# myshell-ai/OpenVoice

Hardware: NVIDIA H100
Metric: audio_seconds_per_second (higher is better)
Workload: dtype f32 (3xFP16 split-precision tensor-core convs with fp32 accumulation, fp32 FFMA elsewhere)

## Files before the change

### openvoice_b200/csrc/ovc_lib.cu

```cuda
#include <cuda_runtime.h>

#include <algorithm>
#include <cmath>
#include <cstdarg>
#include <cstdio>
#include <cstdlib>
#include <cstring>
#include <map>
#include <string>
#include <vector>

#include "../../include/ovc.h"
#include "ovc_convpack.h"
#include "ovc_small.cuh"
#include "ovc_tcconv.cuh"
#include "ovc_tts.cuh"
#include "ovc_refenc.cuh"
#include "ovc_resample.cuh"
#include "ovc_splice.h"
#include "ovc_variants.h"

namespace ovc {

static thread_local std::string g_err;
// ... 116 lines not shown

}

using namespace ovc;

struct ovc_ctx {
  ovc_hparams hp{};
  int device = 0;
  int sm_count = 0;
  std::map<std::string, HostTensor> sd;
  bool finalized = false;

  float* d_w = nullptr;
  size_t w_floats = 0;
  std::vector<float> h_w;

  ConvLayer enc_pre, enc_pre16, enc_proj;
  WNLayers enc_wn;
  ConvLayer flow_pre[4], flow_post[4];
  WNLayers flow_wn[4];
  ConvLayer dec_pre, dec_ups[4];
  ConvLayer rb_c1[12][3], rb_c2[12][3];
  TcLayer tc_c1[12][3], tc_c2[12][3], tc_ups[4], tc_pre;
  float* d_tcw = nullptr;
  std::vector<float> h_tcw;
  int precision = 0;
  bool tts_simple = false;
  bool use_graph = true;
  int use_pdl = 2;
  bool use_branches = true;
  int par_frames = 512;
  bool use_pair = true;
  bool use_pair_occ = true;
  bool use_staged_epi = true;
  bool pair_occ2_ok[TCN_N_OCC2] = {};
  cudaStream_t br_stream[2] = {nullptr, nullptr};
  cudaEvent_t br_ev[4] = {nullptr, nullptr, nullptr, nullptr};
  size_t post_w_off = 0;
  size_t cond_w_off = 0, cond_b_off = 0;
  int* d_cond_wrow = nullptr;
  int* d_cond_sel = nullptr;
  int cond_rows_out = 0;
  int cond_off_enc = 0, cond_off_fsrc = 0, cond_off_ftgt = 0, cond_off_dec = 0;
  int cond_off_enc_tc = 0, cond_off_fsrc_tc = 0, cond_off_ftgt_tc = 0;
  int* d_cond_cols[2][3] = {};
  int cond_pf_cols[2][3] = {};
  int cond_pf_off[2][3][4] = {};

  float2* d_tw = nullptr;
  float* d_win = nullptr;

  bool has_refenc = false;
  size_t re_conv_w[6] = {0}, re_conv_b[6] = {0}, re_wih = 0, re_whh = 0, re_bih = 0, re_bhh = 0, re_pw = 0, re_pb = 0,
         re_lng = 0, re_lnb = 0;
  int re_gru_in = 0;
  float* d_re = nullptr;
  size_t re_floats = 0;
  float* d_res = nullptr;
  size_t res_floats = 0;

  std::map<std::pair<int64_t, int64_t>, double*> rs_banks;
  bool rs_smem_opt_in = false;
  std::vector<RsRingPlan> rs_plans;
  RsRingPlan* d_rs_plans = nullptr;
  int rs_ring_tile = 256;
  size_t rs_ring_smem = 0;

// ... 627 lines not shown
  cfg.dynamicSmemBytes = smem;
  cfg.stream = st;
  cudaLaunchAttribute at[1];
  at[0].id = cudaLaunchAttributeProgrammaticStreamSerialization;
  at[0].val.programmaticStreamSerializationAllowed = 1;
  cfg.attrs = at;
  cfg.numAttrs = pdl ? 1 : 0;
  return cudaLaunchKernelEx(&cfg, kernel, std::forward<Args>(args)...);
}

static int launch_tc(Run& r, const TcLayer& T, const float* x, float* y, const float* res, int t_len, int mul, float slope,
                     float scale, int accumulate, int family, const TcExtra& ex = TcExtra()) {
  TcConvArgs a{};
  const int y_ld = ex.y_ld ? ex.y_ld : T.Ntot;
  a.x = x; a.x_bs = (long long)T.Cin * r.P * mul;
  a.w = reinterpret_cast<const uint16_t*>(r.c->d_tcw + T.w_off);
  a.bias = ex.bias ? ex.bias : r.c->d_tcw + T.b_off; a.bias_bs = ex.bias_bs; a.bias_ts = ex.bias_ts;
  a.y = y; a.y_bs = (long long)y_ld * r.P * mul; a.y_ld = y_ld;
  a.r = res;
  a.s = ex.s; a.s_bs = a.y_bs;
  a.epi = ex.epi; a.split = ex.split; a.first = ex.first;
  a.lens = ex.use_lens_frames ? r.lens : r.glens; a.tmax = r.Tmax; a.mul = mul;
  a.lens_x = ex.lens_x; a.has_lens_x = ex.has_lens_x ? 1 : 0;
  a.Cin = T.Cin; a.Ntot = T.Ntot; a.K = T.K; a.DIL = T.DIL;
  a.slope = slope; a.scale = scale; a.accumulate = accumulate;
  a.passes = r.c->precision == 2 ? 1 : 3;
  if (T.TN == 0) return fail(OVC_ERR_INVALID, "conv %d -> %d (k %d, dilation %d) does not fit the tensor-core kernels", T.Cin, T.Ntot, T.K, T.DIL);
  if (!(slope >= 0.f && slope <= 1.f)) return fail(OVC_ERR_INVALID, "leaky_relu slope %g outside [0, 1]", (double)slope);
  TRY(prof_begin(r));
  const TcGrid g = tc_grid(t_len, r.B, T.Ntot, T.TN, r.c->sm_count, ex.grid_div);
  const int n_tt = g.n_tt, total = g.total;
  dim3 pg((unsigned)g.grid_x, g.ncol, 1);
  const bool pdl = r.c->use_pdl == 1 || (r.c->use_pdl == 2 && ex.epi != 0);
  const TcKernel k = tc_conv_kernel(T.TN, r.c->use_staged_epi && tc_stage_pays(T.K, a.passes));
  CK(launch_ex(k.fn, pg, k.threads, k.smem, r.st, pdl, a, n_tt, total));
  CK(cudaGetLastError());
  r.c->launches++;
  const double units = (double)r.B * t_len;
  const int eff_k = family == 2 ? 2 : T.K;
  TRY(prof_end(r, T.TN == 128 ? V_TC128 : T.TN == 64 ? V_TC64 : V_TC32, family == 1 ? 1 : 0, 2.0 * T.Cin * T.Ntot * eff_k * units,
               4.0 * (T.Cin + T.Ntot * (1 + (res ? 1 : 0) + (accumulate ? 1 : 0))) * units, (T.Cin << 16) | (T.K << 8) | T.DIL));
  return OVC_OK;
}

static int launch_pair(Run& r, const TcLayer& T1, const TcLayer& T2, const float* x, float* y, int t_len, int mul, float slope,
                       float scale, int accumulate) {
  TcConvArgs a{};
  const int C = T1.TN;
  a.x = x; a.x_bs = (long long)C * r.P * mul;
  a.w = reinterpret_cast<const uint16_t*>(r.c->d_tcw + T1.w_off);
  a.w2 = reinterpret_cast<const uint16_t*>(r.c->d_tcw + T2.w_off);
  a.bias = r.c->d_tcw + T1.b_off; a.bias2 = r.c->d_tcw + T2.b_off;
  a.y = y; a.y_bs = a.x_bs; a.y_ld = C;
  a.lens = r.glens; a.tmax = r.Tmax; a.mul = mul;
  a.Cin = C; a.Ntot = C; a.K = T1.K; a.DIL = T1.DIL;
  a.slope = slope; a.scale = scale; a.accumulate = accumulate;
  a.passes = r.c->precision == 2 ? 1 : 3;
  TcPairOcc o = r.c->use_pair_occ ? tc_pair_occ(T1, T2) : TcPairOcc();
  for (int i = 0; i < TCN_N_OCC2; ++i)
    if (o.occ == 2 && kTcPairOcc2[i].C == C && kTcPairOcc2[i].o.nabuf == o.nabuf && !r.c->pair_occ2_ok[i]) o = TcPairOcc();
  const TcKernel k = tc_pair_kernel(C, o, r.c->use_staged_epi && tc_stage_pays(T1.K, a.passes));
  if (!k.fn) return fail(OVC_ERR_INVALID, "no conv-pair kernel for C = %d at %d CTA(s) per SM, %d operand buffer(s)", C, o.occ, o.nabuf);
  const TcGrid g = tc_pair_grid(t_len, r.B, T1.K, r.c->sm_count, o.occ);
  const int n_tt = g.n_tt, total = g.total;
  TRY(prof_begin(r));
  dim3 pg((unsigned)g.grid_x, 1, 1);
  CK(launch_ex(k.fn, pg, k.threads, k.smem, r.st, false, a, n_tt, total));
  CK(cudaGetLastError());
  r.c->launches++;
  const double units = (double)r.B * t_len;
  TRY(prof_end(r, C == 128 ? V_TCPAIR128 : C == 64 ? V_TCPAIR64 : V_TCPAIR32, 1, 2.0 * 2.0 * C * C * T1.K * units, 4.0 * C * (2 + (accumulate ? 1 : 0)) * units,
               (C << 16) | (T1.K << 8) | T1.DIL));
  return OVC_OK;
}

static int launch_transpose(Run& r, const float* src, float* dst, int rows, int cols) {
  dim3 grid((cols + 31) / 32, (rows + 31) / 32, r.B);
  TRY(prof_begin(r));
  transpose_kernel<<<grid, 256, 0, r.st>>>(src, dst, rows, cols, (long long)rows * cols);
  CK(cudaGetLastError());
  r.c->launches++;
  TRY(prof_end(r, V_TRANSPOSE, 0, 0.0, 8.0 * rows * cols * r.B));
  return OVC_OK;
}

struct CondRef {
  const float* p; long long bs, ts;
  CondRef at(int col) const { return {p + col, bs, ts}; }
};

static int run_wn(Run& r, const WNLayers& wn, float* x, float* skip, float* acts, const CondRef& cond) {
  const int P = r.P, T = r.Tmax;
  const long long bs = 192LL * P;
  const int n = (int)wn.in.size();
// ... 1253 lines not shown
  if (!dst || dst_rows < 1 || dst_cap < 1)
    return fail(OVC_ERR_INVALID, "ovc_splice: bad destination (rows %lld, cap %lld)", (long long)dst_rows, (long long)dst_cap);
  if (src_rows < 0 || (src_rows > 0 && (!src || src_pitch < 1)))
    return fail(OVC_ERR_INVALID, "ovc_splice: bad source (rows %lld, pitch %lld)", (long long)src_rows, (long long)src_pitch);
  if (flags & ~(OVC_SPLICE_PCM16 | OVC_SPLICE_SRC_WRAP)) return fail(OVC_ERR_INVALID, "ovc_splice: unknown flags %d", flags);
  if (S == 0) return OVC_OK;
  const int gy = S < 65535 ? S : 65535;
  const int gx = std::max(1, std::min(1024, 2048 / gy));
  ovc_sp::splice_kernel<<<dim3(gx, gy), 256, 0, (cudaStream_t)stream>>>(src, src_rows, src_pitch, seg, S, dst, dst_rows,
                                                                         dst_cap, flags);
  CK(cudaGetLastError());
  return OVC_OK;
}

int ovc_set_precision(ovc_ctx* c, int mode) {
  if (!c) return fail(OVC_ERR_INVALID, "null context");
  if (mode < 0 || mode > 2) return fail(OVC_ERR_INVALID, "precision mode must be 0 (fp32 FFMA), 1 (3xFP16 tensor cores) or 2 (single-pass fp16)");
  c->precision = mode;
  return OVC_OK;
}

int ovc_set_option(ovc_ctx* c, int key, int value) {
  if (!c) return fail(OVC_ERR_INVALID, "null context");
  switch (key) {
    case OVC_OPT_TTS_SIMPLE: c->tts_simple = value != 0; return OVC_OK;
    case OVC_OPT_GRAPH: c->use_graph = value != 0; return OVC_OK;
    case OVC_OPT_PDL:
      if (value < 0 || value > 2) return fail(OVC_ERR_INVALID, "pdl must be 0, 1 or 2");
      c->use_pdl = value;
      return OVC_OK;
    case OVC_OPT_BRANCHES: c->use_branches = value != 0; return OVC_OK;
    case OVC_OPT_PAIR: c->use_pair = value != 0; return OVC_OK;
    case OVC_OPT_PAIR_OCC: c->use_pair_occ = value != 0; return OVC_OK;
    case OVC_OPT_STAGED_EPI: c->use_staged_epi = value != 0; return OVC_OK;
    default: return fail(OVC_ERR_INVALID, "unknown option %d", key);
  }
}

int ovc_last_launch_count(const ovc_ctx* c) { return c ? c->launches : 0; }

int ovc_graph_replays(const ovc_ctx* c) { return c ? c->graph_replays : 0; }

int ovc_profile_enable(ovc_ctx* c, int enable) {
  if (!c) return fail(OVC_ERR_INVALID, "null context");
  c->prof = enable != 0;
  c->ev_used = 0;
  c->ev_flops.clear();
  c->ev_bytes.clear();
  c->ev_variant.clear();
  c->ev_family.clear();
  c->ev_tag.clear();
  return OVC_OK;
}

int ovc_profile_read(ovc_ctx* c, double* ms, int64_t* launches, double* flops, double* bytes) {
  if (!c) return fail(OVC_ERR_INVALID, "null context");
  double tms = 0, tf = 0, tb = 0;
  int64_t n = 0;
  for (size_t i = 0; i + 1 < c->ev_used; i += 2) {
    if (!c->ev_family[i / 2]) continue;
    float m = 0;
    CK(cudaEventElapsedTime(&m, c->ev[i], c->ev[i + 1]));
    tms += m;
    tf += c->ev_flops[i / 2];
    tb += c->ev_bytes[i / 2];
    ++n;
  }
// ... 58 lines not shown
```

### openvoice_b200/csrc/ovc_tcconv.cuh

```cuda
#pragma once
#include "ovc_conv.cuh"
#include "ovc_tc.cuh"
#include "ovc_tcpack.h"

namespace ovc {

struct TcConvArgs {
  const float* x; long long x_bs;
  const uint16_t* w;
  const float* bias; long long bias_bs;
  float* y; long long y_bs; int y_ld;
  const float* r;
  float* s; long long s_bs;
  int epi;
  int split; int first;
  const long long* lens; int tmax; int mul;
  const long long* lens_x; int has_lens_x;
  int Cin; int Ntot; int K; int DIL;
  float slope; float scale; int accumulate;
  int passes;
  const uint16_t* w2; const float* bias2;
  long long bias_ts;
};

// ... 66 lines not shown
      for (int g = 0; g < 2; ++g) {
        const float2 oa = make_float2(tanhf(v[4 * g]) * sigmoidf_acc(v[4 * (g + 2)]),
                                      tanhf(v[4 * g + 1]) * sigmoidf_acc(v[4 * (g + 2) + 1]));
        const float2 ob = make_float2(tanhf(v[4 * g + 2]) * sigmoidf_acc(v[4 * (g + 2) + 2]),
                                      tanhf(v[4 * g + 3]) * sigmoidf_acc(v[4 * (g + 2) + 3]));
        if (oka) *reinterpret_cast<float2*>(ypa + 8 * g) = oa;
        if (okb) *reinterpret_cast<float2*>(ypb + 8 * g) = ob;
      }
    } else {
      const int col = n0 + c0;
      const bool to_x = col < a.split;
      const bool add = to_x || !a.first;
      float* dst = (to_x ? yb + col : sb + (col - a.split)) + csub;
#pragma unroll
      for (int g = 0; g < 4; ++g) {
        float2 oa = make_float2(v[4 * g], v[4 * g + 1]), ob = make_float2(v[4 * g + 2], v[4 * g + 3]);
        if (add) {
          const float2 qa = oka ? *reinterpret_cast<const float2*>(dst + (size_t)ta * a.y_ld + 8 * g) : make_float2(0.f, 0.f);
          const float2 qb = okb ? *reinterpret_cast<const float2*>(dst + (size_t)tb * a.y_ld + 8 * g) : make_float2(0.f, 0.f);
          oa = make_float2(qa.x + oa.x, qa.y + oa.y);
          ob = make_float2(qb.x + ob.x, qb.y + ob.y);
        }
        if (oka) *reinterpret_cast<float2*>(dst + (size_t)ta * a.y_ld + 8 * g) = oa;
        if (okb) *reinterpret_cast<float2*>(dst + (size_t)tb * a.y_ld + 8 * g) = ob;
      }
    }
  }
}

template <int TN, class V>
__device__ __forceinline__ void tc_epilogue_v(const TcConvArgs& a, V v_at, int b, int t0, int n0, int lim, int row_a) {
  if (a.bias_ts) tc_epilogue_body<TN, true>(a, v_at, b, t0, n0, lim, row_a);
  else tc_epilogue_body<TN, false>(a, v_at, b, t0, n0, lim, row_a);
}

template <int TN>
__device__ __forceinline__ void tc_epilogue(const TcConvArgs& a, const float (&d)[TN], int b, int t0, int n0, int lim, int row_a) {
  const bool two = a.passes == 3;
  tc_epilogue_v<TN>(a, [&](int j) { return tc_result<TN>(d, two, j); }, b, t0, n0, lim, row_a);
}
__device__ __forceinline__ TcConvArgs tc_pair_epilogue_args(const TcConvArgs& a, int TN) {
  TcConvArgs e = a;
  e.y_ld = TN; e.r = a.x; e.bias = a.bias2; e.bias_bs = 0; e.bias_ts = 0; e.epi = 0;
  return e;
}

template <int TN>
__device__ __forceinline__ void tc_mma_step(float (&d)[TN], uint64_t a_hi, uint64_t a_lo, uint64_t b, bool three, bool first) {
  float (&lo)[TN / 2] = *reinterpret_cast<float(*)[TN / 2]>(&d[TN / 2]);
  float (&hi)[TN / 2] = *reinterpret_cast<float(*)[TN / 2]>(&d[0]);
  tc::Wgmma<TN>::mma(hi, a_hi, b, first ? 0 : 1);
  if (three) {
    tc::Wgmma<TN>::mma(lo, a_hi, b + TN, first ? 0 : 1);
    tc::Wgmma<TN>::mma(lo, a_lo, b, 1);
  }
}

constexpr int TCN_THREADS = 384;
constexpr int TCN_NCT = 96;

template <int TN, bool PAIR, int OCC = 1, int NAB = 2, bool STAGED = false>
struct TcnCfg {
  static_assert(!PAIR || TN == 32 || TN == 64 || TN == 128, "conv pairs: C = 32, 64 or 128");
  static_assert(OCC == 1 || (PAIR && TN <= 64), "two CTAs per SM: C = 32 / 64 pairs");
  static_assert(!STAGED || (TN == 128 && OCC == 1), "staged epilogue: TN = 128, one CTA per SM");
  static constexpr int THREADS = STAGED ? TCN_THREADS + 128 : TCN_THREADS;
  static constexpr int KCH = 32, NKC = KCH / 8;
  static constexpr int ROWS = 194;
  static constexpr int ROWS2 = TCN_ROWS2;
  static constexpr int NABUF = NAB;
  static constexpr int RING = PAIR ? tc_pair_ring(TN, OCC, NAB) : tc_ring_slots(TN, PAIR);
  static constexpr int SLOT_BYTES = 2 * 2 * TN * 16;
  static constexpr int A_BUF_BYTES = 2 * NKC * ROWS * 16;
  static constexpr int A2_BYTES = PAIR ? 2 * (TN / 8) * ROWS2 * 16 : 0;
  static constexpr int STAGE_BYTES = STAGED ? (TN / 2) * 256 * 4 : 0;
  static_assert(!STAGED || !PAIR || STAGE_BYTES <= A2_BYTES, "a pair's staging tile lies in its conv-2 operand");
  static constexpr int SBUF_BYTES = STAGED && !PAIR ? STAGE_BYTES : 0;
  static constexpr size_t SMEM_BYTES = 1024 + NABUF * A_BUF_BYTES + A2_BYTES + RING * SLOT_BYTES + SBUF_BYTES;
  static_assert(!PAIR || SMEM_BYTES == tc_pair_smem(TN, NABUF, RING), "tc_pair_smem");
  static_assert(SMEM_BYTES <= (OCC == 1 ? 232448 : TCN_SMEM_OCC2), "shared memory budget");
  static_assert((2 * NABUF + 2 * RING + 2) * 8 <= 1024, "barrier area");
  static constexpr int PROD_REGS = OCC == 1 && !STAGED ? 56 : 32, MMA_REGS = STAGED ? 184 : OCC == 1 ? 224 : 104;
  static constexpr int STORE_REGS = 112;
  static_assert(128 * PROD_REGS + 256 * MMA_REGS + (STAGED ? 128 * STORE_REGS : 0) <= 65536 / OCC, "register budget");
};

template <int TN, bool PAIR, int OCC = 1, int NAB = 2, bool STAGED = false>
__global__ void __launch_bounds__(TcnCfg<TN, PAIR, OCC, NAB, STAGED>::THREADS, OCC) tcconv_kernel(const TcConvArgs a, int n_tt, int total) {
  using Cfg = TcnCfg<TN, PAIR, OCC, NAB, STAGED>;
  constexpr int ROWS = Cfg::ROWS, ROWS2 = Cfg::ROWS2, NABUF = Cfg::NABUF, RING = Cfg::RING, NKC = Cfg::NKC;
  extern __shared__ __align__(128) unsigned char smem_raw[];
  uint64_t* bars = reinterpret_cast<uint64_t*>(smem_raw);
  uint64_t *a_full = bars, *a_empty = bars + NABUF, *b_full = a_empty + NABUF, *b_empty = b_full + RING;
  uint64_t *s_full = b_empty + RING, *s_empty = s_full + 1;
  unsigned char* abuf = smem_raw + 1024;
  unsigned char* a2buf = abuf + NABUF * Cfg::A_BUF_BYTES;
  unsigned char* bring = a2buf + Cfg::A2_BYTES;
  float* stage = reinterpret_cast<float*>(PAIR ? a2buf : bring + RING * Cfg::SLOT_BYTES);

  const int tid = threadIdx.x, lane = tid & 31;
  const int warp = __shfl_sync(0xffffffffu, tid >> 5, 0);
  const int H1 = (a.K - 1) / 2 * a.DIL;
  const int H2 = PAIR ? (a.K - 1) / 2 : 0;
  const int R = 128 - 2 * H2;
  const int rows8 = (128 + 2 * H1 + 7) & ~7;
  const int nq = a.Cin / Cfg::KCH;
  const int n_slots = (a.Cin / 16) * a.K;
  const int n_w = PAIR ? 2 * n_slots : n_slots;
  const bool resident = n_w <= RING;
  if (H1 > TCN_HMAX || (PAIR && 128 + 2 * H2 > ROWS2)) __trap();
  constexpr uint32_t BYTES = Cfg::SLOT_BYTES;

  if (tid == 0) {
    for (int i = 0; i < NABUF; ++i) { mbar_init(&a_full[i], TCN_NCT); mbar_init(&a_empty[i], 2); }
    for (int i = 0; i < RING; ++i) { mbar_init(&b_full[i], 1); mbar_init(&b_empty[i], 2); }
    if (STAGED) { mbar_init(s_full, 256); mbar_init(s_empty, 128); }
    fence_mbar_init();
  }
  if (PAIR) {
    for (int i = tid; i < Cfg::A2_BYTES / 16; i += Cfg::THREADS) reinterpret_cast<uint4*>(a2buf)[i] = make_uint4(0u, 0u, 0u, 0u);
// ... 15 lines not shown
    tc::regs_dealloc<Cfg::PROD_REGS>();
    if (warp == 0) {
      if (lane == 0) {
        const unsigned char* wt = reinterpret_cast<const unsigned char*>(a.w) + (size_t)blockIdx.y * n_slots * BYTES;
        if (resident) {
          for (int it = 0; it < n_w; ++it) {
            const unsigned char* src = it < n_slots ? wt + (size_t)it * BYTES
                                                    : reinterpret_cast<const unsigned char*>(a.w2) + (size_t)(it - n_slots) * BYTES;
            mbar_expect_tx(&b_full[it], BYTES);
            tma_bulk_g2s(bring + it * BYTES, src, BYTES, &b_full[it]);
          }
          for (int it = 0; it < n_w; ++it) mbar_wait(&b_full[it], 0u);
        } else {
          int slot = 0;
          uint32_t phase = 1;
          TCN_FOR_TILES
            (void)b;
            for (int it = 0; it < n_w; ++it) {
              const unsigned char* src = it < n_slots ? wt + (size_t)it * BYTES
                                                      : reinterpret_cast<const unsigned char*>(a.w2) + (size_t)(it - n_slots) * BYTES;
              mbar_wait(&b_empty[slot], phase);
              mbar_expect_tx(&b_full[slot], BYTES);
              tma_bulk_g2s(bring + slot * BYTES, src, BYTES, &b_full[slot]);
              if (++slot == RING) { slot = 0; phase ^= 1; }
            }
          }
        }
      }
    } else {
      const int pt = tid - 32;
      const int items = rows8 * NKC;
      int buf = 0;
      uint32_t ephase = 1;
      TCN_FOR_TILES
        const float* xb = a.x + (size_t)b * a.x_bs;
        const int r0 = t0 - H2 - H1;
        for (int q = 0; q < nq; ++q) {
          mbar_wait(&a_empty[buf], ephase);
          unsigned char* ah = abuf + buf * Cfg::A_BUF_BYTES;
          unsigned char* al = ah + NKC * ROWS * 16;
          constexpr int PB = 2;
          for (int i0 = pt; i0 < items; i0 += TCN_NCT * PB) {
            float4 v0[PB], v1[PB];
#pragma unroll
            for (int u = 0; u < PB; ++u) {
              const int i = i0 + TCN_NCT * u;
              const int row = i >> 2, kc = i & 3;
              const int t = r0 + row;
              v0[u] = make_float4(0.f, 0.f, 0.f, 0.f);
              v1[u] = v0[u];
              if (i < items && t >= 0 && t < lim_x) {
                const float4* src = reinterpret_cast<const float4*>(xb + (size_t)t * a.Cin + q * Cfg::KCH + kc * 8);
                v0[u] = src[0];
                v1[u] = src[1];
              }
            }
#pragma unroll
            for (int u = 0; u < PB; ++u) {
              const int i = i0 + TCN_NCT * u;
              if (i >= items) break;
              const int row = i >> 2, kc = i & 3;
              uint4 hi, lo;
              tc::split_f16x8(v0[u], v1[u], a.slope, hi, lo);
              *reinterpret_cast<uint4*>(ah + (kc * ROWS + row) * 16) = hi;
              *reinterpret_cast<uint4*>(al + (kc * ROWS + row) * 16) = lo;
            }
          }
          asm volatile("fence.proxy.async.shared::cta;" ::: "memory");
          mbar_arrive(&a_full[buf]);
          if (++buf == NABUF) { buf = 0; ephase ^= 1; }
        }
      }
    }
  } else if (STAGED && warp >= 12) {
    tc::regs_dealloc<Cfg::STORE_REGS>();
    const int st = tid & 127;
    uint32_t phase = 0;
    TCN_FOR_TILES
      if (PAIR) named_bar_arrive(1, 384);
      mbar_wait(s_full, phase);
      phase ^= 1;
#pragma unroll 1
      for (int h = 0; h < 2; ++h) {
        const float* sv = stage + h * 128 + st;
        const auto v_at = [&](int j) { return sv[j * 256]; };
        const int row_a = 64 * h + 16 * (warp & 3) + (lane >> 2);
        if constexpr (PAIR) tc_epilogue_v<TN>(tc_pair_epilogue_args(a, TN), v_at, b, t0, 0, min(lim, t0 + R), row_a);
        else tc_epilogue_v<TN>(a, v_at, b, t0, blockIdx.y * TN, lim, row_a);
      }
      if (!PAIR) mbar_arrive(s_empty);
    }
  } else {
    tc::regs_alloc<Cfg::MMA_REGS>();
    const int wg = (warp >> 2) - 1;
    const bool leader = (tid & 127) == 0;
    const int row_a = 64 * wg + 16 * (warp & 3) + (lane >> 2);
    constexpr uint32_t LBO_A = ROWS * 16, LBO_A2 = ROWS2 * 16, LBO_B = 2 * TN * 16, SBO = 128;
    constexpr uint32_t A_LO16 = (NKC * ROWS * 16) >> 4, A2_LO16 = ((TN / 8) * ROWS2 * 16) >> 4, SLOT16 = BYTES >> 4;
    const uint64_t a_proto = tc::make_desc(0, LBO_A, SBO), b_proto = tc::make_desc(0, LBO_B, SBO);
    const uint64_t b_ring = b_proto + (tc::smem_addr(bring) >> 4);
    const bool three = a.passes == 3;
    float d[TN];
#pragma unroll
    for (int i = 0; i < TN; ++i) d[i] = 0.f;
    const auto stage_tile = [&]() {
#pragma unroll
      for (int j = 0; j < TN / 2; ++j) stage[j * 256 + tid - 128] = tc_result<TN>(d, three, j);
      mbar_arrive(s_full);
    };
    uint32_t sphase = 1;
    (void)sphase;
    if (resident)
      for (int it = 0; it < n_w; ++it) mbar_wait(&b_full[it], 0u);
    int slot = 0, buf = 0;
    uint32_t bphase = 0, aphase = 0;
    TCN_FOR_TILES
      (void)lim_x;
      bool first = true;
      if (resident) slot = 0;
      for (int q = 0; q < nq; ++q) {
        mbar_wait(&a_full[buf], aphase);
// ... 76 lines not shown
              tc_mma_step<TN>(d, a_cur, a_cur + A2_LO16, b_ring + (uint32_t)slot * SLOT16, three, first2);
              tc::wgmma_commit();
              tc::wgmma_wait<1>();
              if (leader && prev >= 0) mbar_arrive(&b_empty[prev]);
              prev = slot;
              if (++slot == RING) { slot = 0; bphase ^= 1; }
            }
            first2 = false;
            a_cur += 1;
          }
        }
        tc::wgmma_commit();
        tc::wgmma_wait<0>();
        tc::fence_regs(d);
        if (leader && prev >= 0) mbar_arrive(&b_empty[prev]);
        if constexpr (STAGED) {
          named_bar_sync(3, 256);
          stage_tile();
        } else {
          tc_epilogue<TN>(tc_pair_epilogue_args(a, TN), d, b, t0, 0, min(lim, t0 + R), row_a);
        }
      }
    }
  }
#undef TCN_FOR_TILES
}

struct TcKernel {
  void (*fn)(TcConvArgs, int, int) = nullptr;
  size_t smem = 0;
  int threads = 0;
};
using TcPairKernel = TcKernel;
template <int TN, bool PAIR, int OCC = 1, int NAB = 2, bool STAGED = false>
inline TcKernel tc_kernel() {
  using Cfg = TcnCfg<TN, PAIR, OCC, NAB, STAGED>;
  return {tcconv_kernel<TN, PAIR, OCC, NAB, STAGED>, Cfg::SMEM_BYTES, Cfg::THREADS};
}
inline bool tc_stage_pays(int K, int passes) { return passes * K >= 15; }
inline TcKernel tc_conv_kernel(int TN, bool staged) {
  if (TN == 128) return staged ? tc_kernel<128, false, 1, 2, true>() : tc_kernel<128, false>();
  if (TN == 64) return tc_kernel<64, false>();
  if (TN == 32) return tc_kernel<32, false>();
  return {};
}
inline TcKernel tc_pair_kernel(int C, TcPairOcc o, bool staged = false) {
  if (o.occ == 1 && o.nabuf == 2) {
    if (C == 128) return staged ? tc_kernel<128, true, 1, 2, true>() : tc_kernel<128, true>();
    if (C == 64) return tc_kernel<64, true>();
    if (C == 32) return tc_kernel<32, true>();
  } else if (o.occ == 2) {
    if (C == 32 && o.nabuf == 2) return tc_kernel<32, true, 2, 2>();
    if (C == 32 && o.nabuf == 1) return tc_kernel<32, true, 2, 1>();
    if (C == 64 && o.nabuf == 1) return tc_kernel<64, true, 2, 1>();
  }
  return {};
}
constexpr int TCN_N_OCC2 = 3;
constexpr struct { int C; TcPairOcc o; } kTcPairOcc2[TCN_N_OCC2] = {{32, {2, 2}}, {32, {2, 1}}, {64, {2, 1}}};

template <int C>
__global__ void __launch_bounds__(256) conv_post_cl_kernel(const float* __restrict__ x, long long x_bs,
                                                           const float* __restrict__ w, float* __restrict__ y,
                                                           long long y_bs, int y_len, const long long* lens, int tmax,
                                                           int mul) {
  constexpr int TB = 256, ROWS = TB + 6, LD = ROWS + 3;
  __shared__ float ws[7][C];
  __shared__ float xs[C][LD];
  for (int i = threadIdx.x; i < C * 7; i += blockDim.x) ws[i % 7][i / 7] = w[i];
  const int b = blockIdx.y;
  const int lim = (lens ? (int)min((long long)tmax, lens[b]) : tmax) * mul;
  const int t0 = blockIdx.x * TB;
  const float* xb = x + (size_t)b * x_bs;
  for (int idx = threadIdx.x; idx < ROWS * (C / 4); idx += blockDim.x) {
// ... 43 lines not shown
```

### openvoice_b200/csrc/ovc_tcpack.h

```cpp
#pragma once
#include <cuda_fp16.h>
#include <stddef.h>
#include <stdint.h>

#include <algorithm>

namespace ovc {

constexpr int TCN_HMAX = 25;
constexpr int TCN_ROWS2 = 146;

constexpr int tc_ring_slots(int TN, bool pair) {
  return pair ? (TN == 32 ? 44 : TN == 64 ? 24 : 12) : (TN == 32 ? 22 : 12);
}

struct TcGeom {
  int Cin = 0, Ntot = 0, K = 0, DIL = 1, TN = 0;
};

inline int tc_tile_n(int Ntot, int Cin, int K, int DIL) {
  if (Ntot <= 0 || Cin <= 0 || K <= 0 || DIL <= 0) return 0;
  if (Ntot % 32 || Cin % 32 || (K - 1) / 2 * DIL > TCN_HMAX) return 0;
  return Ntot % 128 == 0 ? 128 : (Ntot % 64 == 0 ? 64 : 32);
}

inline size_t tc_slot_halfs(int TN) { return (size_t)2 * 2 * TN * 8; }
inline size_t tc_packed_halfs(int Ntot, int Cin, int K, int TN) {
  return TN ? (size_t)(Ntot / TN) * (Cin / 16) * K * tc_slot_halfs(TN) : 0;
}
inline size_t tc_packed_index(int Cin, int K, int TN, int n, int ci, int tap, int part) {
  const int nt = n / TN, k16 = ci / 16, kc = (ci % 16) / 8, e = ci % 8;
  const size_t slot = ((size_t)nt * (Cin / 16) + k16) * K + tap;
  return slot * tc_slot_halfs(TN) + ((size_t)(kc * 2 + part) * TN + n % TN) * 8 + e;
}

inline void tc_split(float w, uint16_t& hi, uint16_t& lo) {
  const __half h = __float2half_rn(w);
  const __half l = __float2half_rn((w - __half2float(h)) * 2048.f);
  hi = __half_as_ushort(h);
  lo = __half_as_ushort(l);
}

template <class WF>
inline void tc_pack_weights(uint16_t* dst, int Ntot, int Cin, int K, int TN, WF wfun) {
  for (int nt = 0; nt < Ntot / TN; ++nt)
    for (int k16 = 0; k16 < Cin / 16; ++k16)
      for (int tap = 0; tap < K; ++tap) {
// ... 30 lines not shown
         T2.DIL == 1 && (T1.K - 1) / 2 * T1.DIL <= TCN_HMAX && 128 + 2 * ((T2.K - 1) / 2) <= TCN_ROWS2;
}

struct TcGrid {
  int n_tt = 0, total = 0, grid_x = 0, ncol = 0;
};
inline TcGrid tc_grid(int t_len, int B, int Ntot, int TN, int sm_count, int grid_div) {
  TcGrid g;
  g.n_tt = (t_len + 127) / 128;
  g.total = g.n_tt * B;
  g.ncol = Ntot / TN;
  const int per_col = std::max(1, sm_count / g.ncol / std::max(1, grid_div));
  g.grid_x = std::min(g.total, per_col);
  return g;
}
inline TcGrid tc_pair_grid(int t_len, int B, int K, int sm_count, int occ = 1) {
  TcGrid g;
  const int R = 128 - (K - 1);
  g.n_tt = (t_len + R - 1) / R;
  g.total = g.n_tt * B;
  g.ncol = 1;
  g.grid_x = std::min(g.total, occ * sm_count);
  return g;
}

constexpr size_t tc_pair_smem(int TN, int nabuf, int ring) {
  return 1024 + (size_t)nabuf * 2 * 4 * 194 * 16 + (size_t)2 * (TN / 8) * TCN_ROWS2 * 16 + (size_t)ring * 2 * 2 * TN * 16;
}
constexpr size_t TCN_SMEM_OCC2 = (233472 - 2 * 1024) / 2;
constexpr int tc_pair_ring(int TN, int occ, int nabuf) {
  return occ == 1 ? tc_ring_slots(TN, true) : (int)((TCN_SMEM_OCC2 - tc_pair_smem(TN, nabuf, 0)) / (2 * 2 * TN * 16));
}

struct TcPairOcc {
  int occ = 1, nabuf = 2;
};
inline TcPairOcc tc_pair_occ(const TcGeom& T1, const TcGeom& T2) {
  TcPairOcc o;
  if (!tc_pair_fuses(T1, T2)) return o;
  const int n_w = 2 * (T1.Cin / 16) * T1.K;
  if (T1.TN == 32 && n_w <= tc_pair_ring(32, 2, 2)) o = {2, 2};
  else if (T1.TN == 32 && n_w <= tc_pair_ring(32, 2, 1)) o = {2, 1};
  else if (T1.TN == 64 && n_w > tc_pair_ring(64, 1, 2)) o = {2, 1};
  return o;
}

}
```

### openvoice_b200/csrc/ovc_conv.cuh

```cuda
#pragma once
#include <cuda_runtime.h>
#include <stdint.h>

namespace ovc {

enum EpiKind : int {
  EPI_LINEAR = 0,
  EPI_GATE = 1,
  EPI_RESSKIP = 2,
  EPI_PROJ = 3,
  EPI_COUPLE = 4,
  EPI_UPS8 = 5,
  EPI_UPS2 = 6
};

enum : int { F_ACCUM = 1, F_FIRST = 2 };

struct ItemParams {
  const unsigned long long* seed; const long long* stream; const long long* frame0;
  const float* tau; const float* noise_scale; const float* noise_scale_w; const float* length_scale; const float* sdp_ratio;
};

struct CallParams { unsigned long long seed; float tau; float pad; ItemParams items; };

// ... 34 lines not shown
  uint32_t ok;
  asm volatile(
      "{\n\t.reg .pred p;\n\t"
      "mbarrier.try_wait.parity.shared::cta.b64 p, [%1], %2;\n\t"
      "selp.u32 %0, 1, 0, p;\n\t}"
      : "=r"(ok)
      : "r"(smem_u32(bar)), "r"(parity)
      : "memory");
  return ok != 0;
}
__device__ __forceinline__ void mbar_wait(uint64_t* bar, uint32_t parity) {
  if (mbar_try_wait(bar, parity)) return;
  const long long t0 = clock64();
  while (!mbar_try_wait(bar, parity)) {
    if (clock64() - t0 > 4000000000LL) __trap();
  }
}
__device__ __forceinline__ void tma_bulk_g2s(void* dst, const void* src, uint32_t bytes, uint64_t* bar) {
  asm volatile(
      "cp.async.bulk.shared::cluster.global.mbarrier::complete_tx::bytes [%0], [%1], %2, [%3];" ::"r"(
          smem_u32(dst)),
      "l"(src), "r"(bytes), "r"(smem_u32(bar))
      : "memory");
}
__device__ __forceinline__ void cp_async16_zfill(void* dst, const void* src, uint32_t src_bytes) {
  asm volatile("cp.async.cg.shared.global [%0], [%1], 16, %2;" ::"r"(smem_u32(dst)), "l"(src), "r"(src_bytes)
               : "memory");
}
__device__ __forceinline__ void cp_async4_zfill(void* dst, const void* src, uint32_t src_bytes) {
  asm volatile("cp.async.ca.shared.global [%0], [%1], 4, %2;" ::"r"(smem_u32(dst)), "l"(src), "r"(src_bytes)
               : "memory");
}
__device__ __forceinline__ void cp_async_wait_all() { asm volatile("cp.async.wait_all;" ::: "memory"); }

__device__ __forceinline__ float lrelu(float v, float slope) { return v > 0.f ? v : v * slope; }
__device__ __forceinline__ float sigmoidf_acc(float v) { return 1.f / (1.f + expf(-v)); }

__device__ __forceinline__ float philox_normal(unsigned long long seed, uint32_t c0, uint32_t c1, uint32_t c2) {
  uint32_t k0 = static_cast<uint32_t>(seed), k1 = static_cast<uint32_t>(seed >> 32);
  uint32_t x0 = c0, x1 = c1, x2 = c2, x3 = 0x0B200u;
#pragma unroll
  for (int i = 0; i < 10; ++i) {
    const uint32_t hi0 = __umulhi(0xD2511F53u, x0), lo0 = 0xD2511F53u * x0;
    const uint32_t hi1 = __umulhi(0xCD9E8D57u, x2), lo1 = 0xCD9E8D57u * x2;
    const uint32_t y0 = hi1 ^ x1 ^ k0, y1 = lo1, y2 = hi0 ^ x3 ^ k1, y3 = lo0;
    x0 = y0; x1 = y1; x2 = y2; x3 = y3;
    k0 += 0x9E3779B9u; k1 += 0xBB67AE85u;
  }
  const float u1 = (static_cast<float>(x0 >> 8) + 0.5f) * (1.0f / 16777216.0f);
  const float u2 = (static_cast<float>(x1 >> 8) + 0.5f) * (1.0f / 16777216.0f);
  return sqrtf(-2.0f * logf(u1)) * cospif(2.0f * u2);
}

__host__ __device__ constexpr int floor4(int v) { return v >= 0 ? (v / 4) * 4 : -(((-v) + 3) / 4) * 4; }

template <int K, int DIL, int NG>
struct TapGeom {
  static constexpr int HALF = (K - 1) / 2;
  static constexpr int TPG = (K + NG - 1) / NG;
  __host__ __device__ static constexpr int off(int k) { return (k - HALF) * DIL; }
  __host__ __device__ static constexpr int k_lo(int g) { return g * TPG; }
  __host__ __device__ static constexpr int k_hi(int g) { return (g + 1) * TPG < K ? (g + 1) * TPG : K; }
  __host__ __device__ static constexpr int lo(int g) { return floor4(off(k_lo(g))); }
  __host__ __device__ static constexpr int nvec(int g) { return (off(k_hi(g) - 1) + 3 - lo(g)) / 4 + 1; }
  static constexpr int HL = -lo(0);
  static constexpr int HR = lo(NG - 1) + 4 * nvec(NG - 1) - 4;
// ... 420 lines not shown
```

Baseline: 2423.

## Batch epilogue loads, add L2 bulk prefetch of residuals, widen staged-epilogue use

Adds a new staged epilogue that loads the residual, accumulator and split inputs for whole 32-column groups before doing the arithmetic. A dedicated warp issues cp.async.bulk L2 prefetches for those epilogue inputs while the MMA for the tile is still running. The rule that decides when the staged epilogue is used changes: with 3 passes it now triggers for K>=5, and with single-pass precision it is used only for pairs. A mode 2 can force it on. The goal is to hide the epilogue's global-memory latency, at the cost of extra register pressure and extra prefetch traffic.

```diff
diff --git a/openvoice_b200/csrc/ovc_lib.cu b/openvoice_b200/csrc/ovc_lib.cu
--- a/openvoice_b200/csrc/ovc_lib.cu
+++ b/openvoice_b200/csrc/ovc_lib.cu
@@ -172,7 +172,7 @@
   int par_frames = 512;
   bool use_pair = true;
   bool use_pair_occ = true;
-  bool use_staged_epi = true;
+  int use_staged_epi = 1;
   bool pair_occ2_ok[TCN_N_OCC2] = {};
   cudaStream_t br_stream[2] = {nullptr, nullptr};
   cudaEvent_t br_ev[4] = {nullptr, nullptr, nullptr, nullptr};
@@ -866,7 +866,7 @@
   const int n_tt = g.n_tt, total = g.total;
   dim3 pg((unsigned)g.grid_x, g.ncol, 1);
   const bool pdl = r.c->use_pdl == 1 || (r.c->use_pdl == 2 && ex.epi != 0);
-  const TcKernel k = tc_conv_kernel(T.TN, r.c->use_staged_epi && tc_stage_pays(T.K, a.passes));
+  const TcKernel k = tc_conv_kernel(T.TN, r.c->use_staged_epi == 2 || (r.c->use_staged_epi && tc_stage_pays(T.K, a.passes, false)));
   CK(launch_ex(k.fn, pg, k.threads, k.smem, r.st, pdl, a, n_tt, total));
   CK(cudaGetLastError());
   r.c->launches++;
@@ -893,7 +893,7 @@
   TcPairOcc o = r.c->use_pair_occ ? tc_pair_occ(T1, T2) : TcPairOcc();
   for (int i = 0; i < TCN_N_OCC2; ++i)
     if (o.occ == 2 && kTcPairOcc2[i].C == C && kTcPairOcc2[i].o.nabuf == o.nabuf && !r.c->pair_occ2_ok[i]) o = TcPairOcc();
-  const TcKernel k = tc_pair_kernel(C, o, r.c->use_staged_epi && tc_stage_pays(T1.K, a.passes));
+  const TcKernel k = tc_pair_kernel(C, o, r.c->use_staged_epi == 2 || (r.c->use_staged_epi && tc_stage_pays(T1.K, a.passes, true)));
   if (!k.fn) return fail(OVC_ERR_INVALID, "no conv-pair kernel for C = %d at %d CTA(s) per SM, %d operand buffer(s)", C, o.occ, o.nabuf);
   const TcGrid g = tc_pair_grid(t_len, r.B, T1.K, r.c->sm_count, o.occ);
   const int n_tt = g.n_tt, total = g.total;
@@ -2213,7 +2213,10 @@
     case OVC_OPT_BRANCHES: c->use_branches = value != 0; return OVC_OK;
     case OVC_OPT_PAIR: c->use_pair = value != 0; return OVC_OK;
     case OVC_OPT_PAIR_OCC: c->use_pair_occ = value != 0; return OVC_OK;
-    case OVC_OPT_STAGED_EPI: c->use_staged_epi = value != 0; return OVC_OK;
+    case OVC_OPT_STAGED_EPI:
+      if (value < 0 || value > 2) return fail(OVC_ERR_INVALID, "staged_epi must be 0, 1 or 2");
+      c->use_staged_epi = value;
+      return OVC_OK;
     default: return fail(OVC_ERR_INVALID, "unknown option %d", key);
   }
 }
diff --git a/openvoice_b200/csrc/ovc_tcconv.cuh b/openvoice_b200/csrc/ovc_tcconv.cuh
--- a/openvoice_b200/csrc/ovc_tcconv.cuh
+++ b/openvoice_b200/csrc/ovc_tcconv.cuh
@@ -122,6 +122,146 @@
 __device__ __forceinline__ void tc_epilogue_v(const TcConvArgs& a, V v_at, int b, int t0, int n0, int lim, int row_a) {
   if (a.bias_ts) tc_epilogue_body<TN, true>(a, v_at, b, t0, n0, lim, row_a);
   else tc_epilogue_body<TN, false>(a, v_at, b, t0, n0, lim, row_a);
+}
+
+template <int TN, bool PF, int GB, class V>
+__device__ __forceinline__ void tc_store_epilogue_body(const TcConvArgs& a, V v_at, int b, int t0, int n0, int lim, int row_a) {
+  static_assert(TN % (32 * GB) == 0, "whole batches of 32-column groups");
+  const int csub = (threadIdx.x & 3) * 2;
+  float* yb = a.y + (size_t)b * a.y_bs;
+  const float* rb = a.r ? a.r + (size_t)b * a.y_bs : nullptr;
+  float* sb = a.s ? a.s + (size_t)b * a.s_bs : nullptr;
+  const int ta = t0 + row_a, tb = ta + 8;
+  const bool oka = ta < lim, okb = tb < lim;
+  const float* bias_a = a.bias + (size_t)b * a.bias_bs + (PF ? (size_t)min(ta, a.tmax - 1) * a.bias_ts : 0);
+  const float* bias_b = a.bias + (size_t)b * a.bias_bs + (PF ? (size_t)min(tb, a.tmax - 1) * a.bias_ts : 0);
+  const float2 z = make_float2(0.f, 0.f);
+  const auto ld2 = [](const float* p, bool ok) { return ok ? *reinterpret_cast<const float2*>(p) : make_float2(0.f, 0.f); };
+#pragma unroll 1
+  for (int c1 = 0; c1 < TN; c1 += 32 * GB) {
+    float2 p[GB][4][2], q[GB][4][2];
+#pragma unroll
+    for (int u = 0; u < GB; ++u) {
+      const int c0 = c1 + 32 * u;
+#pragma unroll
+      for (int g = 0; g < 4; ++g) {
+        p[u][g][0] = p[u][g][1] = q[u][g][0] = q[u][g][1] = z;
+        if (a.epi == 0) {
+          const size_t off = (size_t)n0 + c0 + csub + 8 * g;
+          if (rb) { p[u][g][0] = ld2(rb + (size_t)ta * a.y_ld + off, oka); p[u][g][1] = ld2(rb + (size_t)tb * a.y_ld + off, okb); }
+          if (a.accumulate) { q[u][g][0] = ld2(yb + (size_t)ta * a.y_ld + off, oka); q[u][g][1] = ld2(yb + (size_t)tb * a.y_ld + off, okb); }
+        } else if (a.epi == 2) {
+          const int col = n0 + c0;
+          const bool to_x = col < a.split;
+          if (to_x || !a.first) {
+            const float* src = (to_x ? yb + col : sb + (col - a.split)) + csub + 8 * g;
+            p[u][g][0] = ld2(src + (size_t)ta * a.y_ld, oka);
+            p[u][g][1] = ld2(src + (size_t)tb * a.y_ld, okb);
+          }
+        }
+      }
+    }
+#pragma unroll
+    for (int u = 0; u < GB; ++u) {
+      const int c0 = c1 + 32 * u;
+      float v[16];
+#pragma unroll
+      for (int i = 0; i < 16; ++i) v[i] = v_at(c0 / 2 + i);
+#pragma unroll
+      for (int g = 0; g < 4; ++g) {
+        const float2 bq = __ldg(reinterpret_cast<const float2*>(bias_a + n0 + c0 + 8 * g + csub));
+        const float2 br = PF ? __ldg(reinterpret_cast<const float2*>(bias_b + n0 + c0 + 8 * g + csub)) : bq;
+        v[4 * g] += bq.x; v[4 * g + 1] += bq.y; v[4 * g + 2] += br.x; v[4 * g + 3] += br.y;
+      }
+      if (a.epi == 0) {
+        float* ypa = yb + (size_t)ta * a.y_ld + n0 + c0 + csub;
+        float* ypb = yb + (size_t)tb * a.y_ld + n0 + c0 + csub;
+#pragma unroll
+        for (int g = 0; g < 4; ++g) {
+          float2 oa = make_float2(v[4 * g], v[4 * g + 1]), ob = make_float2(v[4 * g + 2], v[4 * g + 3]);
+          if (rb) {
+            const float2 qa = p[u][g][0], qb = p[u][g][1];
+            oa.x += qa.x; oa.y += qa.y; ob.x += qb.x; ob.y += qb.y;
+          }
+          if (a.accumulate) {
+            const float2 ya = q[u][g][0], yc = q[u][g][1];
+            oa.x = ya.x + oa.x; oa.y = ya.y + oa.y;
+            ob.x = yc.x + ob.x; ob.y = yc.y + ob.y;
+          }
+          if (a.scale != 1.f) { oa.x *= a.scale; oa.y *= a.scale; ob.x *= a.scale; ob.y *= a.scale; }
+          if (oka) *reinterpret_cast<float2*>(ypa + 8 * g) = oa;
+          if (okb) *reinterpret_cast<float2*>(ypb + 8 * g) = ob;
+        }
+      } else if (a.epi == 1) {
+        float* ypa = yb + (size_t)ta * a.y_ld + ((n0 + c0) >> 1) + csub;
+        float* ypb = yb + (size_t)tb * a.y_ld + ((n0 + c0) >> 1) + csub;
+#pragma unroll
+        for (int g = 0; g < 2; ++g) {
+          const float2 oa = make_float2(tanhf(v[4 * g]) * sigmoidf_acc(v[4 * (g + 2)]),
+                                        tanhf(v[4 * g + 1]) * sigmoidf_acc(v[4 * (g + 2) + 1]));
+          const float2 ob = make_float2(tanhf(v[4 * g + 2]) * sigmoidf_acc(v[4 * (g + 2) + 2]),
+                                        tanhf(v[4 * g + 3]) * sigmoidf_acc(v[4 * (g + 2) + 3]));
+          if (oka) *reinterpret_cast<float2*>(ypa + 8 * g) = oa;
+          if (okb) *reinterpret_cast<float2*>(ypb + 8 * g) = ob;
+        }
+      } else {
+        const int col = n0 + c0;
+        const bool to_x = col < a.split;
+        const bool add = to_x || !a.first;
+        float* dst = (to_x ? yb + col : sb + (col - a.split)) + csub;
+#pragma unroll
+        for (int g = 0; g < 4; ++g) {
+          float2 oa = make_float2(v[4 * g], v[4 * g + 1]), ob = make_float2(v[4 * g + 2], v[4 * g + 3]);
+          if (add) {
+            const float2 qa = p[u][g][0], qb = p[u][g][1];
+            oa = make_float2(qa.x + oa.x, qa.y + oa.y);
+            ob = make_float2(qb.x + ob.x, qb.y + ob.y);
+          }
+          if (oka) *reinterpret_cast<float2*>(dst + (size_t)ta * a.y_ld + 8 * g) = oa;
+          if (okb) *reinterpret_cast<float2*>(dst + (size_t)tb * a.y_ld + 8 * g) = ob;
+        }
+      }
+    }
+  }
+}
+
+template <int TN, class V>
+__device__ __forceinline__ void tc_store_epilogue_v(const TcConvArgs& a, V v_at, int b, int t0, int n0, int lim, int row_a) {
+  constexpr int GB = TN / 32 < 2 ? TN / 32 : 2;
+  if (a.bias_ts) tc_store_epilogue_body<TN, true, GB>(a, v_at, b, t0, n0, lim, row_a);
+  else tc_store_epilogue_body<TN, false, GB>(a, v_at, b, t0, n0, lim, row_a);
+}
+
+__device__ __forceinline__ void l2_prefetch_bulk(const void* p, uint32_t bytes) {
+  if (bytes == 0 || (((uintptr_t)p | bytes) & 15)) return;
+  asm volatile("cp.async.bulk.prefetch.L2.global [%0], %1;" ::"l"(p), "r"(bytes) : "memory");
+}
+
+template <int TN, bool PAIR>
+__device__ __forceinline__ void tc_store_prefetch(const TcConvArgs& a, int b, int t0, int t1, int n0, int lane) {
+  if (t1 <= t0 || a.epi == 1) return;
+  const float* yb = a.y + (size_t)b * a.y_bs;
+  if constexpr (PAIR) {
+    if (lane == 0) {
+      const uint32_t bytes = (uint32_t)(t1 - t0) * TN * 4;
+      l2_prefetch_bulk(a.x + (size_t)b * a.x_bs + (size_t)t0 * TN, bytes);
+      if (a.accumulate) l2_prefetch_bulk(yb + (size_t)t0 * TN, bytes);
+    }
+  } else {
+    const float* rb = a.r ? a.r + (size_t)b * a.y_bs : nullptr;
+    const float* sb = a.s ? a.s + (size_t)b * a.s_bs : nullptr;
+    const int xc = a.epi == 2 ? min(max(a.split - n0, 0), TN) : TN;
+    for (int t = t0 + lane; t < t1; t += 32) {
+      const size_t row = (size_t)t * a.y_ld;
+      if (a.epi == 0) {
+        if (rb) l2_prefetch_bulk(rb + row + n0, TN * 4);
+        if (a.accumulate) l2_prefetch_bulk(yb + row + n0, TN * 4);
+      } else {
+        l2_prefetch_bulk(yb + row + n0, (uint32_t)xc * 4);
+        if (!a.first && xc < TN) l2_prefetch_bulk(sb + row + (n0 + xc - a.split), (uint32_t)(TN - xc) * 4);
+      }
+    }
+  }
 }
 
 template <int TN>
@@ -302,6 +442,8 @@
     const int st = tid & 127;
     uint32_t phase = 0;
     TCN_FOR_TILES
+      const int t1 = PAIR ? min(lim, t0 + R) : min(lim, t0 + 128);
+      if (warp == 12) tc_store_prefetch<TN, PAIR>(a, b, t0, t1, PAIR ? 0 : blockIdx.y * TN, lane);
       if (PAIR) named_bar_arrive(1, 384);
       mbar_wait(s_full, phase);
       phase ^= 1;
@@ -310,8 +452,8 @@
         const float* sv = stage + h * 128 + st;
         const auto v_at = [&](int j) { return sv[j * 256]; };
         const int row_a = 64 * h + 16 * (warp & 3) + (lane >> 2);
-        if constexpr (PAIR) tc_epilogue_v<TN>(tc_pair_epilogue_args(a, TN), v_at, b, t0, 0, min(lim, t0 + R), row_a);
-        else tc_epilogue_v<TN>(a, v_at, b, t0, blockIdx.y * TN, lim, row_a);
+        if constexpr (PAIR) tc_store_epilogue_v<TN>(tc_pair_epilogue_args(a, TN), v_at, b, t0, 0, t1, row_a);
+        else tc_store_epilogue_v<TN>(a, v_at, b, t0, blockIdx.y * TN, lim, row_a);
       }
       if (!PAIR) mbar_arrive(s_empty);
     }
@@ -459,7 +601,6 @@
   using Cfg = TcnCfg<TN, PAIR, OCC, NAB, STAGED>;
   return {tcconv_kernel<TN, PAIR, OCC, NAB, STAGED>, Cfg::SMEM_BYTES, Cfg::THREADS};
 }
-inline bool tc_stage_pays(int K, int passes) { return passes * K >= 15; }
 inline TcKernel tc_conv_kernel(int TN, bool staged) {
   if (TN == 128) return staged ? tc_kernel<128, false, 1, 2, true>() : tc_kernel<128, false>();
   if (TN == 64) return tc_kernel<64, false>();
diff --git a/openvoice_b200/csrc/ovc_tcpack.h b/openvoice_b200/csrc/ovc_tcpack.h
--- a/openvoice_b200/csrc/ovc_tcpack.h
+++ b/openvoice_b200/csrc/ovc_tcpack.h
@@ -109,6 +109,8 @@
   return occ == 1 ? tc_ring_slots(TN, true) : (int)((TCN_SMEM_OCC2 - tc_pair_smem(TN, nabuf, 0)) / (2 * 2 * TN * 16));
 }
 
+inline bool tc_stage_pays(int K, int passes, bool pair = false) { return passes == 3 ? K >= 5 : pair; }
+
 struct TcPairOcc {
   int occ = 1, nabuf = 2;
 };
```

Result: no change. 2410, median of 6 (-0.5%).

## Land conv operands with cp.async lookahead before in-place fp16 split

Applied to the files above, without the earlier changes.

For non-pair tensor-core convs, the producer warps now issue cp.async copies of raw fp32 input rows straight into the operand buffers. They convert older buffers in place to hi/lo fp16 only after a lookahead of several groups, instead of loading into registers and splitting synchronously. Non-staged convs get four operand buffers instead of two so that loads for later chunks overlap conversion of earlier ones. The cost is more shared memory per CTA and a conversion pass that reads from and writes back to shared memory.

```diff
diff --git a/openvoice_b200/csrc/ovc_conv.cuh b/openvoice_b200/csrc/ovc_conv.cuh
--- a/openvoice_b200/csrc/ovc_conv.cuh
+++ b/openvoice_b200/csrc/ovc_conv.cuh
@@ -90,6 +90,9 @@
                : "memory");
 }
 __device__ __forceinline__ void cp_async_wait_all() { asm volatile("cp.async.wait_all;" ::: "memory"); }
+__device__ __forceinline__ void cp_async_commit() { asm volatile("cp.async.commit_group;" ::: "memory"); }
+template <int N>
+__device__ __forceinline__ void cp_async_wait_group() { asm volatile("cp.async.wait_group %0;" ::"n"(N) : "memory"); }
 
 __device__ __forceinline__ float lrelu(float v, float slope) { return v > 0.f ? v : v * slope; }
 __device__ __forceinline__ float sigmoidf_acc(float v) { return 1.f / (1.f + expf(-v)); }
diff --git a/openvoice_b200/csrc/ovc_tcconv.cuh b/openvoice_b200/csrc/ovc_tcconv.cuh
--- a/openvoice_b200/csrc/ovc_tcconv.cuh
+++ b/openvoice_b200/csrc/ovc_tcconv.cuh
@@ -149,7 +149,7 @@
 constexpr int TCN_THREADS = 384;
 constexpr int TCN_NCT = 96;
 
-template <int TN, bool PAIR, int OCC = 1, int NAB = 2, bool STAGED = false>
+template <int TN, bool PAIR, int OCC = 1, int NAB = PAIR ? 2 : tc_conv_nabuf(false), bool STAGED = false>
 struct TcnCfg {
   static_assert(!PAIR || TN == 32 || TN == 64 || TN == 128, "conv pairs: C = 32, 64 or 128");
   static_assert(OCC == 1 || (PAIR && TN <= 64), "two CTAs per SM: C = 32 / 64 pairs");
@@ -159,6 +159,9 @@
   static constexpr int ROWS = 194;
   static constexpr int ROWS2 = TCN_ROWS2;
   static constexpr int NABUF = NAB;
+  static constexpr bool LANDING = !PAIR;
+  static constexpr int LOOK = NABUF - 1;
+  static_assert(!LANDING || LOOK >= 1, "landing: two operand buffers at least");
   static constexpr int RING = PAIR ? tc_pair_ring(TN, OCC, NAB) : tc_ring_slots(TN, PAIR);
   static constexpr int SLOT_BYTES = 2 * 2 * TN * 16;
   static constexpr int A_BUF_BYTES = 2 * NKC * ROWS * 16;
@@ -175,7 +178,7 @@
   static_assert(128 * PROD_REGS + 256 * MMA_REGS + (STAGED ? 128 * STORE_REGS : 0) <= 65536 / OCC, "register budget");
 };
 
-template <int TN, bool PAIR, int OCC = 1, int NAB = 2, bool STAGED = false>
+template <int TN, bool PAIR, int OCC = 1, int NAB = PAIR ? 2 : tc_conv_nabuf(false), bool STAGED = false>
 __global__ void __launch_bounds__(TcnCfg<TN, PAIR, OCC, NAB, STAGED>::THREADS, OCC) tcconv_kernel(const TcConvArgs a, int n_tt, int total) {
   using Cfg = TcnCfg<TN, PAIR, OCC, NAB, STAGED>;
   constexpr int ROWS = Cfg::ROWS, ROWS2 = Cfg::ROWS2, NABUF = Cfg::NABUF, RING = Cfg::RING, NKC = Cfg::NKC;
@@ -257,43 +260,91 @@
       const int items = rows8 * NKC;
       int buf = 0;
       uint32_t ephase = 1;
-      TCN_FOR_TILES
-        const float* xb = a.x + (size_t)b * a.x_bs;
-        const int r0 = t0 - H2 - H1;
-        for (int q = 0; q < nq; ++q) {
-          mbar_wait(&a_empty[buf], ephase);
-          unsigned char* ah = abuf + buf * Cfg::A_BUF_BYTES;
+      if constexpr (Cfg::LANDING) {
+        constexpr int LOOK = Cfg::LOOK;
+        int cbuf = 0, pending = 0;
+        const auto convert_oldest = [&]() {
+          unsigned char* ah = abuf + cbuf * Cfg::A_BUF_BYTES;
           unsigned char* al = ah + NKC * ROWS * 16;
-          constexpr int PB = 2;
-          for (int i0 = pt; i0 < items; i0 += TCN_NCT * PB) {
-            float4 v0[PB], v1[PB];
-#pragma unroll
-            for (int u = 0; u < PB; ++u) {
-              const int i = i0 + TCN_NCT * u;
+          for (int i = pt; i < items; i += TCN_NCT) {
+            const int row = i >> 2, kc = i & 3;
+            unsigned char* ph = ah + (kc * ROWS + row) * 16;
+            unsigned char* pl = al + (kc * ROWS + row) * 16;
+            uint4 hi, lo;
+            tc::split_f16x8(*reinterpret_cast<const float4*>(ph), *reinterpret_cast<const float4*>(pl), a.slope, hi, lo);
+            *reinterpret_cast<uint4*>(ph) = hi;
+            *reinterpret_cast<uint4*>(pl) = lo;
+          }
+          asm volatile("fence.proxy.async.shared::cta;" ::: "memory");
+          mbar_arrive(&a_full[cbuf]);
+          if (++cbuf == NABUF) cbuf = 0;
+          --pending;
+        };
+        TCN_FOR_TILES
+          const float* xb = a.x + (size_t)b * a.x_bs;
+          const int r0 = t0 - H2 - H1;
+          for (int q = 0; q < nq; ++q) {
+            if (pending == LOOK) {
+              cp_async_wait_group<LOOK - 1>();
+              convert_oldest();
+            }
+            mbar_wait(&a_empty[buf], ephase);
+            unsigned char* ah = abuf + buf * Cfg::A_BUF_BYTES;
+            unsigned char* al = ah + NKC * ROWS * 16;
+            for (int i = pt; i < items; i += TCN_NCT) {
               const int row = i >> 2, kc = i & 3;
               const int t = r0 + row;
-              v0[u] = make_float4(0.f, 0.f, 0.f, 0.f);
-              v1[u] = v0[u];
-              if (i < items && t >= 0 && t < lim_x) {
-                const float4* src = reinterpret_cast<const float4*>(xb + (size_t)t * a.Cin + q * Cfg::KCH + kc * 8);
-                v0[u] = src[0];
-                v1[u] = src[1];
+              const bool ok = t >= 0 && t < lim_x;
+              const float* src = ok ? xb + (size_t)t * a.Cin + q * Cfg::KCH + kc * 8 : a.x;
+              cp_async16_zfill(ah + (kc * ROWS + row) * 16, src, ok ? 16u : 0u);
+              cp_async16_zfill(al + (kc * ROWS + row) * 16, src + (ok ? 4 : 0), ok ? 16u : 0u);
+            }
+            cp_async_commit();
+            ++pending;
+            if (++buf == NABUF) { buf = 0; ephase ^= 1; }
+          }
+        }
+        cp_async_wait_all();
+        while (pending) convert_oldest();
+      } else {
+        TCN_FOR_TILES
+          const float* xb = a.x + (size_t)b * a.x_bs;
+          const int r0 = t0 - H2 - H1;
+          for (int q = 0; q < nq; ++q) {
+            mbar_wait(&a_empty[buf], ephase);
+            unsigned char* ah = abuf + buf * Cfg::A_BUF_BYTES;
+            unsigned char* al = ah + NKC * ROWS * 16;
+            constexpr int PB = 2;
+            for (int i0 = pt; i0 < items; i0 += TCN_NCT * PB) {
+              float4 v0[PB], v1[PB];
+#pragma unroll
+              for (int u = 0; u < PB; ++u) {
+                const int i = i0 + TCN_NCT * u;
+                const int row = i >> 2, kc = i & 3;
+                const int t = r0 + row;
+                v0[u] = make_float4(0.f, 0.f, 0.f, 0.f);
+                v1[u] = v0[u];
+                if (i < items && t >= 0 && t < lim_x) {
+                  const float4* src = reinterpret_cast<const float4*>(xb + (size_t)t * a.Cin + q * Cfg::KCH + kc * 8);
+                  v0[u] = src[0];
+                  v1[u] = src[1];
+                }
+              }
+#pragma unroll
+              for (int u = 0; u < PB; ++u) {
+                const int i = i0 + TCN_NCT * u;
+                if (i >= items) break;
+                const int row = i >> 2, kc = i & 3;
+                uint4 hi, lo;
+                tc::split_f16x8(v0[u], v1[u], a.slope, hi, lo);
+                *reinterpret_cast<uint4*>(ah + (kc * ROWS + row) * 16) = hi;
+                *reinterpret_cast<uint4*>(al + (kc * ROWS + row) * 16) = lo;
               }
             }
-#pragma unroll
-            for (int u = 0; u < PB; ++u) {
-              const int i = i0 + TCN_NCT * u;
-              if (i >= items) break;
-              const int row = i >> 2, kc = i & 3;
-              uint4 hi, lo;
-              tc::split_f16x8(v0[u], v1[u], a.slope, hi, lo);
-              *reinterpret_cast<uint4*>(ah + (kc * ROWS + row) * 16) = hi;
-              *reinterpret_cast<uint4*>(al + (kc * ROWS + row) * 16) = lo;
-            }
-          }
-          asm volatile("fence.proxy.async.shared::cta;" ::: "memory");
-          mbar_arrive(&a_full[buf]);
-          if (++buf == NABUF) { buf = 0; ephase ^= 1; }
+            asm volatile("fence.proxy.async.shared::cta;" ::: "memory");
+            mbar_arrive(&a_full[buf]);
+            if (++buf == NABUF) { buf = 0; ephase ^= 1; }
+          }
         }
       }
     }
@@ -454,14 +505,14 @@
   int threads = 0;
 };
 using TcPairKernel = TcKernel;
-template <int TN, bool PAIR, int OCC = 1, int NAB = 2, bool STAGED = false>
+template <int TN, bool PAIR, int OCC = 1, int NAB = PAIR ? 2 : tc_conv_nabuf(false), bool STAGED = false>
 inline TcKernel tc_kernel() {
   using Cfg = TcnCfg<TN, PAIR, OCC, NAB, STAGED>;
   return {tcconv_kernel<TN, PAIR, OCC, NAB, STAGED>, Cfg::SMEM_BYTES, Cfg::THREADS};
 }
 inline bool tc_stage_pays(int K, int passes) { return passes * K >= 15; }
 inline TcKernel tc_conv_kernel(int TN, bool staged) {
-  if (TN == 128) return staged ? tc_kernel<128, false, 1, 2, true>() : tc_kernel<128, false>();
+  if (TN == 128) return staged ? tc_kernel<128, false, 1, tc_conv_nabuf(true), true>() : tc_kernel<128, false>();
   if (TN == 64) return tc_kernel<64, false>();
   if (TN == 32) return tc_kernel<32, false>();
   return {};
diff --git a/openvoice_b200/csrc/ovc_tcpack.h b/openvoice_b200/csrc/ovc_tcpack.h
--- a/openvoice_b200/csrc/ovc_tcpack.h
+++ b/openvoice_b200/csrc/ovc_tcpack.h
@@ -13,6 +13,8 @@
 constexpr int tc_ring_slots(int TN, bool pair) {
   return pair ? (TN == 32 ? 44 : TN == 64 ? 24 : 12) : (TN == 32 ? 22 : 12);
 }
+
+constexpr int tc_conv_nabuf(bool staged) { return staged ? 2 : 4; }
 
 struct TcGeom {
   int Cin = 0, Ntot = 0, K = 0, DIL = 1, TN = 0;
```

After: 2387 before, 2400 after, median of 6. About the same (+0.6%).
